# facebookresearch/vilbert-multi-task

Measured on AMD Instinct MI355X. Metric: samples/sec (36 regions, 36 tokens) ViLBERT-base 6L/6C fwd+bwd, higher is better.
Workload: dtype f32; 1 GPU; bert_base_6layer_6conect.json train_concap step: BertForMultiModalPreTraining fwd+bwd (dropout on) + grad all-reduce + AdamW, 36 regions + 1 global row, batch 256 per GPU, T=36 R=37; per_gpu_batch=256, global_batch=256, parallelism=dp1, visible_gpus=1, launch=eager, gemm_mode=f32, deterministic_wgrad=True, deterministic_fallbacks=0

## Files before the change

vilbert-multi-task_amd/csrc/common.h:

```cpp
#pragma once
#include <hip/hip_runtime.h>
#include <stdint.h>

#include "bf16_round.h"
#include "gemm_plan.h"
#include "row_checks.h"

typedef float f32x4 __attribute__((ext_vector_type(4)));
typedef float f32x16 __attribute__((ext_vector_type(16)));

#define VB_LAUNCH_CHECK()                         \
    do {                                          \
        hipError_t e__ = hipGetLastError();       \
        if (e__ != hipSuccess) return (int)e__;   \
    } while (0)

const uint64_t* vb_seed_epoch();

namespace vbemb {
int text_embed_bwd_det(hipStream_t st, int batch, int n_tok, int hidden, int vocab, int n_types, int n_tasks,
                       const int64_t* ids, const int64_t* seg, const int64_t* task_ids, const float* dx, float* dword,
                       float* dpos, float* dtype, float* dtask);
}

namespace vbrows {
int gather(hipStream_t st, long M, int cols, const float* src, const int32_t* map, long src_rows, float* out);
int drop_add(hipStream_t st, long M, int cols, const float* lin, const float* res, bool res_mapped, const int32_t* map,
             long src_rows, float* out, float p, uint64_t seed);
int invert(hipStream_t st, long src_rows, long M, const int32_t* map, int32_t* inv);
int scatter(hipStream_t st, long src_rows, int cols, const float* compact, long M, const int32_t* inv, float* full);
int move_rows(hipStream_t st, long rows, int chunks, const void* src, long lds, long src_rows, const int32_t* map, void* out,
              long ldo, long max_blocks);
int colsum_finish(hipStream_t st, long parts, int n, const float* part, long ldp, float* out);
}

__device__ __forceinline__ float wave_sum(float v) {
#pragma unroll
    for (int off = 32; off > 0; off >>= 1) v += __shfl_xor(v, off, 64);
    return v;
}

__device__ __forceinline__ void gelu_parts(float x, float& phi, float& e) {
    const float z = fabsf(x) * 0.70710678118654752440f;
    const float t = __builtin_amdgcn_rcpf(fmaf(0.3275911f, z, 1.0f));
    e = __expf(-z * z);
    float poly = fmaf(1.061405429f, t, -1.453152027f);
    poly = fmaf(poly, t, 1.421413741f);
    poly = fmaf(poly, t, -0.284496736f);
    poly = fmaf(poly, t, 0.254829592f);
    const float half_erfc = 0.5f * poly * t * e;
    phi = x >= 0.f ? 1.0f - half_erfc : half_erfc;
}

__device__ __forceinline__ float gelu_erf(float x) {
    float phi, e;
    gelu_parts(x, phi, e);
    return x * phi;
}

__device__ __forceinline__ float gelu_grad(float x) {
    float phi, e;
    gelu_parts(x, phi, e);
    return fmaf(x * 0.39894228040143267794f, e, phi);
}

__device__ __forceinline__ void gelu_and_grad(float x, float& y, float& d) {
    float phi, e;
    gelu_parts(x, phi, e);
    y = x * phi;
    d = fmaf(x * 0.39894228040143267794f, e, phi);
}

__device__ __forceinline__ float swish_act(float x) {
    return x / (1.0f + expf(-x));
}

__device__ __forceinline__ float swish_grad(float x) {
    const float s = 1.0f / (1.0f + expf(-x));
    return s + x * s * (1.0f - s);
}
```

vilbert-multi-task_amd/csrc/layernorm.hip:

```cpp
#include "rowops.h"
#include "rng.h"

using namespace vbrow;

namespace {

template <int NV>
__global__ __launch_bounds__(256) void layernorm_kernel(long rows, int n_cols, const float* __restrict__ x,
                                                        const float* __restrict__ x2,
                                                        const float* __restrict__ gamma,
                                                        const float* __restrict__ beta, float eps,
                                                        float* __restrict__ y, float* mean, float* rstd,
                                                        unsigned char* __restrict__ q, long ldq,
                                                        float* __restrict__ qscale, unsigned* __restrict__ mxs,
                                                        long mxs_rows) {
    const int lane = threadIdx.x & 63;
    const long row = (long)blockIdx.x * ROWS_PER_BLOCK + (threadIdx.x >> 6);
    if (row >= rows) return;
    const float* xr = x + row * n_cols;
    f32x4 v[NV];
#pragma unroll
    for (int i = 0; i < NV; ++i) {
        const int col = VB_LANE_COL(i, lane);
        v[i] = f32x4{0.f, 0.f, 0.f, 0.f};
        if (col < n_cols) {
            v[i] = *reinterpret_cast<const f32x4*>(xr + col);
            if (x2 != nullptr) v[i] += *reinterpret_cast<const f32x4*>(x2 + row * n_cols + col);
        }
    }
    ln_finish<NV>(v, n_cols, lane, gamma, beta, eps, y + row * n_cols, mean ? mean + row : nullptr,
                  rstd ? rstd + row : nullptr, nullptr, q ? q + row * ldq : nullptr, (q && qscale) ? qscale + row : nullptr,
                  mxs ? mxs + row : nullptr, mxs_rows);
}

struct EmitStats {
    static constexpr bool MX = false;
    float* __restrict__ mean;
    float* __restrict__ rstd;
};
struct EmitMX {
    static constexpr bool MX = true;
    unsigned char* __restrict__ q;
    long ldq;
    unsigned* __restrict__ mxs;
    long mxs_rows;
};

__device__ __forceinline__ f32x4 ln16_value(const uint2 w, const f32x4 g, const f32x4 b, float mean, float rstd) {
    return g * ((RowBF16::unpack(w) - mean) * rstd) + b;
}

template <int NV, int R, typename Emit>
__global__ __launch_bounds__(256) void layernorm16_kernel(long rows, int n_cols, const unsigned short* __restrict__ x,
                                                          const float* __restrict__ gamma, const float* __restrict__ beta,
                                                          float eps, unsigned short* __restrict__ y, const Emit out) {
    using IO = RowBF16;
    const int lane = threadIdx.x & 63;
    const long row0 = ((long)blockIdx.x * ROWS_PER_BLOCK + (threadIdx.x >> 6)) * R;
    if (row0 >= rows) return;
    long rrow[R];
    bool have[R];
#pragma unroll
    for (int r = 0; r < R; ++r) {
        have[r] = row0 + r < rows;
        rrow[r] = have[r] ? row0 + r : row0;
    }
    uint2 w[R][NV];
#pragma unroll
    for (int r = 0; r < R; ++r)
#pragma unroll
        for (int i = 0; i < NV; ++i) {
            const int col = VB_LANE_COL(i, lane);
            w[r][i] = uint2{0u, 0u};
            if (col < n_cols) w[r][i] = *reinterpret_cast<const uint2*>(x + rrow[r] * n_cols + col);
        }
    auto opaque = [&]() {
#pragma unroll
        for (int r = 0; r < R; ++r)
#pragma unroll
            for (int i = 0; i < NV; ++i) asm volatile("" : "+v"(w[r][i].x), "+v"(w[r][i].y));
    };
    float mu[R], q[R];
#pragma unroll
    for (int r = 0; r < R; ++r) {
        mu[r] = 0.f;
#pragma unroll
        for (int i = 0; i < NV; ++i) {
            const f32x4 v = IO::unpack(w[r][i]);
            mu[r] += (v[0] + v[1]) + (v[2] + v[3]);
        }
    }
    wave_sum_rows(mu);
    if (R > 1) opaque();
#pragma unroll
    for (int r = 0; r < R; ++r) {
        mu[r] /= (float)n_cols;
        q[r] = 0.f;
#pragma unroll
        for (int i = 0; i < NV; ++i) {
            const int col = VB_LANE_COL(i, lane);
            if (col < n_cols) {
                const f32x4 d = IO::unpack(w[r][i]) - mu[r];
                q[r] += (d[0] * d[0] + d[1] * d[1]) + (d[2] * d[2] + d[3] * d[3]);
            }
        }
    }
    wave_sum_rows(q);
    if (R > 1) opaque();
    if constexpr (!Emit::MX) {
#pragma unroll
        for (int r = 0; r < R; ++r) {
            q[r] = 1.0f / sqrtf(q[r] / (float)n_cols + eps);
            if (lane == 0 && have[r]) {
                if (out.mean != nullptr) out.mean[rrow[r]] = mu[r];
                if (out.rstd != nullptr) out.rstd[rrow[r]] = q[r];
            }
        }
#pragma unroll
        for (int i = 0; i < NV; ++i) {
            const int col = VB_LANE_COL(i, lane);
            if (col < n_cols) {
                const f32x4 g = *reinterpret_cast<const f32x4*>(gamma + col), b = *reinterpret_cast<const f32x4*>(beta + col);
#pragma unroll
                for (int r = 0; r < R; ++r)
                    if (have[r]) IO::store(y + rrow[r] * n_cols + col, ln16_value(w[r][i], g, b, mu[r], q[r]));
            }
        }
    } else {
        const int nkt = n_cols >> 7;
#pragma unroll
        for (int i = 0; i < NV; ++i) {
            const int col = VB_LANE_COL(i, lane);
            const bool ok = col < n_cols;
            f32x4 g = f32x4{0.f, 0.f, 0.f, 0.f}, b = f32x4{0.f, 0.f, 0.f, 0.f};
            if (ok) {
                g = *reinterpret_cast<const f32x4*>(gamma + col);
                b = *reinterpret_cast<const f32x4*>(beta + col);
            }
            const int kt = 2 * i + (lane >> 5);
#pragma unroll
            for (int r = 0; r < R; ++r) {
                const float rstd = 1.0f / sqrtf(q[r] / (float)n_cols + eps);
                const bool live = ok && have[r];
                f32x4 v = IO::unpack(w[r][i]);
                if (ok) v = ln16_value(w[r][i], g, b, mu[r], rstd);
                if (live) IO::store(y + rrow[r] * n_cols + col, v);
                mx_quant_chunk(v, live, lane, have[r] ? kt : nkt, nkt,
                               reinterpret_cast<unsigned*>(out.q + rrow[r] * out.ldq + (ok ? col : 0)),
                               out.mxs + (long)(kt < nkt ? kt : 0) * out.mxs_rows + rrow[r]);
            }
        }
    }
}

constexpr int LNB_ROWS_PER_WAVE = 4;
constexpr int LNB_ROWS_PER_BLOCK = 4 * LNB_ROWS_PER_WAVE;

inline long lnb_blocks(long rows) { return (rows + LNB_ROWS_PER_BLOCK - 1) / LNB_ROWS_PER_BLOCK; }

template <int NV, typename IO>
__global__ __launch_bounds__(256) void layernorm_bwd_kernel(long rows, int n_cols, const typename IO::elem* __restrict__ dy,
                                                            const typename IO::elem* __restrict__ x,
                                                            const float* __restrict__ mean, const float* __restrict__ rstd,
                                                            const float* __restrict__ gamma,
                                                            typename IO::elem* __restrict__ dx, float* __restrict__ ws,
                                                            typename IO::elem* __restrict__ dxd, float drop_p,
                                                            float drop_scale, uint64_t seed_in,
                                                            const uint64_t* __restrict__ epoch) {
    const uint64_t seed = dxd != nullptr ? vb_seed_with_epoch(seed_in, epoch) : 0;
    const int lane = threadIdx.x & 63, wave = threadIdx.x >> 6;
    const long part = (long)blockIdx.x * 4 + wave;
    const long row_begin = part * LNB_ROWS_PER_WAVE;
    f32x4 gam[NV], dg[NV], db[NV];
#pragma unroll
    for (int i = 0; i < NV; ++i) {
        const int col = VB_LANE_COL(i, lane);
        gam[i] = col < n_cols ? *reinterpret_cast<const f32x4*>(gamma + col) : f32x4{0.f, 0.f, 0.f, 0.f};
        dg[i] = f32x4{0.f, 0.f, 0.f, 0.f};
        db[i] = f32x4{0.f, 0.f, 0.f, 0.f};
    }
    [[maybe_unused]] typename IO::packed ndy[NV], nx[NV];
    [[maybe_unused]] float nmu = 0.f, nrs = 0.f;
    [[maybe_unused]] auto fetch = [&](long row) {
#pragma unroll
        for (int i = 0; i < NV; ++i) {
            const int col = VB_LANE_COL(i, lane);
            ndy[i] = IO::zero();
            nx[i] = IO::zero();
            if (col < n_cols) {
                ndy[i] = *reinterpret_cast<const typename IO::packed*>(dy + row * n_cols + col);
                nx[i] = *reinterpret_cast<const typename IO::packed*>(x + row * n_cols + col);
            }
        }
        nmu = mean[row];
        nrs = rstd[row];
    };
    if constexpr (IO::PREFETCH)
        if (row_begin < rows) fetch(row_begin);
    for (int rr = 0; rr < LNB_ROWS_PER_WAVE; ++rr) {
        const long row = row_begin + rr;
        if (row >= rows) break;
        const float mu = IO::PREFETCH ? nmu : mean[row], rs = IO::PREFETCH ? nrs : rstd[row];
        f32x4 xh[NV], g[NV];
        [[maybe_unused]] f32x4 dcur[NV];
        if constexpr (IO::PREFETCH) {
#pragma unroll
            for (int i = 0; i < NV; ++i) {
                dcur[i] = IO::unpack(ndy[i]);
                xh[i] = IO::unpack(nx[i]);
            }
            if (rr + 1 < LNB_ROWS_PER_WAVE && row + 1 < rows) fetch(row + 1);
        }
        float s1 = 0.f, s2 = 0.f;
#pragma unroll
        for (int i = 0; i < NV; ++i) {
            const int col = VB_LANE_COL(i, lane);
            if constexpr (!IO::PREFETCH) xh[i] = f32x4{0.f, 0.f, 0.f, 0.f};
            g[i] = f32x4{0.f, 0.f, 0.f, 0.f};
            if (col < n_cols) {
                const f32x4 d = IO::PREFETCH ? dcur[i] : *reinterpret_cast<const f32x4*>(dy + row * n_cols + col);
                xh[i] = ((IO::PREFETCH ? xh[i] : *reinterpret_cast<const f32x4*>(x + row * n_cols + col)) - mu) * rs;
                g[i] = d * gam[i];
                dg[i] += d * xh[i];
                db[i] += d;
                s1 += (g[i][0] + g[i][1]) + (g[i][2] + g[i][3]);
                s2 += (g[i][0] * xh[i][0] + g[i][1] * xh[i][1]) + (g[i][2] * xh[i][2] + g[i][3] * xh[i][3]);
            }
        }
        const float m1 = wave_sum(s1) / (float)n_cols, m2 = wave_sum(s2) / (float)n_cols;
#pragma unroll
        for (int i = 0; i < NV; ++i) {
            const int col = VB_LANE_COL(i, lane);
            if (col < n_cols) {
                const f32x4 d = (g[i] - m1 - xh[i] * m2) * rs;
                IO::store(dx + row * n_cols + col, d);
                if (dxd != nullptr) {
                    f32x4 dd;
                    const uint64_t idx = (uint64_t)(row * n_cols + col);
#pragma unroll
                    for (int e = 0; e < 4; ++e) dd[e] = vb_keep(seed, idx + e, drop_p) ? d[e] * drop_scale : 0.f;
                    IO::store(dxd + row * n_cols + col, dd);
                }
            }
        }
    }
    constexpr bool BLOCK_REDUCE = NV <= 4;
    __shared__ f32x4 red[BLOCK_REDUCE ? 3 * 2 * NV * 64 : 1];
    if (BLOCK_REDUCE) {
        if (wave > 0) {
#pragma unroll
            for (int i = 0; i < NV; ++i) {
                red[((wave - 1) * 2 * NV + i) * 64 + lane] = dg[i];
                red[((wave - 1) * 2 * NV + NV + i) * 64 + lane] = db[i];
            }
        }
        __syncthreads();
        if (wave > 0) return;
#pragma unroll
        for (int w2 = 0; w2 < 3; ++w2)
#pragma unroll
            for (int i = 0; i < NV; ++i) {
                dg[i] += red[(w2 * 2 * NV + i) * 64 + lane];
                db[i] += red[(w2 * 2 * NV + NV + i) * 64 + lane];
            }
    }
    float* w = ws + (BLOCK_REDUCE ? (long)blockIdx.x : part) * 2 * n_cols;
#pragma unroll
    for (int i = 0; i < NV; ++i) {
        const int col = VB_LANE_COL(i, lane);
        if (col < n_cols) {
            *reinterpret_cast<f32x4*>(w + col) = dg[i];
            *reinterpret_cast<f32x4*>(w + n_cols + col) = db[i];
        }
    }
}

__global__ __launch_bounds__(256) void layernorm_bwd_wide_kernel(long rows, int n_cols, const float* __restrict__ dy,
                                                                 const float* __restrict__ x,
                                                                 const float* __restrict__ mean,
                                                                 const float* __restrict__ rstd,
                                                                 const float* __restrict__ gamma,
                                                                 float* __restrict__ dx, float* __restrict__ ws) {
    const int lane = threadIdx.x & 63;
    const long row = (long)blockIdx.x * 4 + (threadIdx.x >> 6);
    if (row >= rows) return;
    const float mu = mean[row], rs = rstd[row];
    const float* __restrict__ dyr = dy + row * n_cols;
    const float* __restrict__ xr = x + row * n_cols;
    float s1 = 0.f, s2 = 0.f;
    for (int col = lane * 4; col < n_cols; col += 256) {
        const f32x4 d = *reinterpret_cast<const f32x4*>(dyr + col);
        const f32x4 xh = (*reinterpret_cast<const f32x4*>(xr + col) - mu) * rs;
        const f32x4 g = d * *reinterpret_cast<const f32x4*>(gamma + col);
        s1 += (g[0] + g[1]) + (g[2] + g[3]);
        s2 += (g[0] * xh[0] + g[1] * xh[1]) + (g[2] * xh[2] + g[3] * xh[3]);
    }
    const float m1 = wave_sum(s1) / (float)n_cols, m2 = wave_sum(s2) / (float)n_cols;
    float* __restrict__ w = ws + row * 2 * n_cols;
    for (int col = lane * 4; col < n_cols; col += 256) {
        const f32x4 d = *reinterpret_cast<const f32x4*>(dyr + col);
        const f32x4 xh = (*reinterpret_cast<const f32x4*>(xr + col) - mu) * rs;
        const f32x4 g = d * *reinterpret_cast<const f32x4*>(gamma + col);
        *reinterpret_cast<f32x4*>(dx + row * n_cols + col) = (g - m1 - xh * m2) * rs;
        *reinterpret_cast<f32x4*>(w + col) = d * xh;
        *reinterpret_cast<f32x4*>(w + n_cols + col) = d;
    }
}

template <int INFLIGHT>
__global__ __launch_bounds__(1024) void colreduce_kernel(long parts, int width, const float* __restrict__ ws,
                                                         float* __restrict__ out0, float* __restrict__ out1, int n_cols) {
    static_assert(INFLIGHT == 1 || INFLIGHT == 4, "instantiated forms");
    __shared__ float red[16][INFLIGHT == 1 ? 64 : 65];
    const int c = threadIdx.x & 63, pg = threadIdx.x >> 6;
    const int col = blockIdx.x * 64 + c;
    float s0 = 0.f, s1 = 0.f, s2 = 0.f, s3 = 0.f;
    if (col < width) {
        long p = pg;
        if constexpr (INFLIGHT == 4)
            for (; p + 48 < parts; p += 64) {
                s0 += ws[p * width + col];
                s1 += ws[(p + 16) * width + col];
                s2 += ws[(p + 32) * width + col];
                s3 += ws[(p + 48) * width + col];
            }
        for (; p < parts; p += 16) s0 += ws[p * width + col];
    }
    red[pg][c] = INFLIGHT == 4 ? (s0 + s1) + (s2 + s3) : s0;
    __syncthreads();
    if (pg == 0 && col < width) {
        float t = 0.f;
#pragma unroll
        for (int i = 0; i < 16; ++i) t += red[i][c];
        if (col < n_cols) out0[col] = t;
        else out1[col - n_cols] = t;
    }
}

template <int INFLIGHT>
int launch_colreduce(hipStream_t st, long parts, int n_cols, const float* ws, float* dgamma, float* dbeta) {
    const int width = 2 * n_cols;
    hipLaunchKernelGGL(colreduce_kernel<INFLIGHT>, dim3((unsigned)((width + 63) / 64)), dim3(1024), 0, st, parts, width, ws,
                       dgamma, dbeta, n_cols);
    VB_LAUNCH_CHECK();
    return 0;
}

inline bool codes_ok(const void* q, int64_t ldq, int n_cols) { return ldq >= n_cols && ldq % 4 == 0 && all_aligned(4, {q}); }

int launch_layernorm(void* stream, int64_t rows, int32_t n_cols, const float* x, const float* x2, const float* gamma,
                     const float* beta, float eps, float* y, float* mean, float* rstd, uint8_t* q, int64_t ldq,
                     float* qscale, uint32_t* mxs, int64_t mxs_rows) {
    if (!all_aligned(16, {x, x2, y, gamma, beta}) || (q != nullptr && !codes_ok(q, ldq, n_cols)) || !all_aligned(4, {mxs}))
        return VB_E_ALIGN;
    const dim3 grid((unsigned)((rows + ROWS_PER_BLOCK - 1) / ROWS_PER_BLOCK)), block(256);
    dispatch_nv<32>(nv_for(n_cols), [&](auto nv) {
        hipLaunchKernelGGL((layernorm_kernel<decltype(nv)::value>), grid, block, 0, static_cast<hipStream_t>(stream), (long)rows,
                           n_cols, x, x2, gamma, beta, eps, y, mean, rstd, q, (long)ldq, qscale, mxs, (long)mxs_rows);
    });
    VB_LAUNCH_CHECK();
    return 0;
}

template <int R, int MAX, typename Emit>
void launch_layernorm16(void* stream, int64_t rows, int32_t n_cols, const uint16_t* x, const float* gamma, const float* beta,
                        float eps, uint16_t* y, const Emit out) {
    const dim3 grid((unsigned)((rows + R * ROWS_PER_BLOCK - 1) / (R * ROWS_PER_BLOCK))), block(256);
    dispatch_nv<MAX>(nv_for(n_cols), [&](auto nv) {
        hipLaunchKernelGGL((layernorm16_kernel<decltype(nv)::value, R, Emit>), grid, block, 0, static_cast<hipStream_t>(stream),
                           (long)rows, n_cols, x, gamma, beta, eps, y, out);
    });
}

template <typename IO, int MAX, int INFLIGHT>
int layernorm_bwd_impl(void* stream, int64_t rows, int32_t n_cols, const typename IO::elem* dy, const typename IO::elem* x,
                       const float* mean, const float* rstd, const float* gamma, typename IO::elem* dx, float* dgamma,
                       float* dbeta, float* workspace, typename IO::elem* dxd, float drop_p, uint64_t seed) {
    if (!all_aligned(IO::ALIGN, {dy, x, dx, dxd}) || !all_aligned(16, {gamma, workspace})) return VB_E_ALIGN;
    hipStream_t st = static_cast<hipStream_t>(stream);
    const long blocks = lnb_blocks(rows);
    const float dscale = dxd != nullptr ? 1.0f / (1.0f - drop_p) : 1.0f;
    const uint64_t* epoch = vb_seed_epoch();
    dispatch_nv<MAX>(nv_for(n_cols), [&](auto nv) {
        hipLaunchKernelGGL((layernorm_bwd_kernel<decltype(nv)::value, IO>), dim3((unsigned)blocks), dim3(256), 0, st, (long)rows,
                           n_cols, dy, x, mean, rstd, gamma, dx, workspace, dxd, drop_p, dscale, seed, epoch);
    });
    VB_LAUNCH_CHECK();
    return launch_colreduce<INFLIGHT>(st, nv_for(n_cols) <= 4 ? blocks : blocks * 4, n_cols, workspace, dgamma, dbeta);
}

int layernorm_bwd_f32(void* stream, int64_t rows, int32_t n_cols, const float* dy, const float* x, const float* mean,
                      const float* rstd, const float* gamma, float* dx, float* dgamma, float* dbeta, float* workspace,
                      float* dxd, float drop_p, uint64_t seed) {
    if (any_null({dy, x, mean, rstd, gamma, dx, dgamma, dbeta, workspace}) || rows <= 0) return VB_E_BADARG;
    if (int e = check_cols(n_cols)) return e;
    if (nv_for(n_cols) <= 16)
        return layernorm_bwd_impl<RowF32, 16, 1>(stream, rows, n_cols, dy, x, mean, rstd, gamma, dx, dgamma, dbeta, workspace,
                                                 dxd, drop_p, seed);
    if (!all_aligned(16, {dy, x, dx, gamma, workspace})) return VB_E_ALIGN;
    if (dxd != nullptr) return VB_E_RANGE;
    hipStream_t st = static_cast<hipStream_t>(stream);
    hipLaunchKernelGGL(layernorm_bwd_wide_kernel, dim3((unsigned)((rows + 3) / 4)), dim3(256), 0, st, (long)rows, n_cols, dy, x,
                       mean, rstd, gamma, dx, workspace);
    VB_LAUNCH_CHECK();
    return launch_colreduce<1>(st, rows, n_cols, workspace, dgamma, dbeta);
}

}

extern "C" int vb_layernorm_fwd(void* stream, int64_t rows, int32_t n_cols, const float* x, const float* x2,
                                const float* gamma, const float* beta, float eps, float* y, float* mean,
                                float* rstd) {
    if (any_null({x, gamma, beta, y}) || rows <= 0) return VB_E_BADARG;
    if (int e = check_cols(n_cols)) return e;
    return launch_layernorm(stream, rows, n_cols, x, x2, gamma, beta, eps, y, mean, rstd, nullptr, 0, nullptr, nullptr, 0);
}

extern "C" int vb_layernorm_fwd_fp8(void* stream, int64_t rows, int32_t n_cols, const float* x, const float* x2,
                                    const float* gamma, const float* beta, float eps, float* y, uint8_t* q,
                                    int64_t ldq, float* qscale) {
    if (any_null({x, gamma, beta, y, q, qscale}) || rows <= 0) return VB_E_BADARG;
    if (int e = check_cols(n_cols)) return e;
    return launch_layernorm(stream, rows, n_cols, x, x2, gamma, beta, eps, y, nullptr, nullptr, q, ldq, qscale, nullptr, 0);
}

extern "C" int vb_layernorm_fwd_mx(void* stream, int64_t rows, int32_t n_cols, const float* x, const float* x2,
                                   const float* gamma, const float* beta, float eps, float* y, uint8_t* q, int64_t ldq,
                                   uint32_t* scales, int64_t scale_rows) {
    if (any_null({x, gamma, beta, y, q, scales}) || rows <= 0) return VB_E_BADARG;
    if (int e = check_cols(n_cols)) return e;
    if (n_cols % 128 != 0 || scale_rows < rows) return VB_E_RANGE;
    return launch_layernorm(stream, rows, n_cols, x, x2, gamma, beta, eps, y, nullptr, nullptr, q, ldq, nullptr, scales,
                            scale_rows);
}

extern "C" int vb_layernorm_fwd_mx16(void* stream, int64_t rows, int32_t n_cols, const uint16_t* x, const float* gamma,
                                     const float* beta, float eps, uint16_t* y, uint8_t* q, int64_t ldq, uint32_t* scales,
                                     int64_t scale_rows) {
    if (any_null({x, gamma, beta, y, q, scales}) || rows <= 0) return VB_E_BADARG;
    if (int e = check_cols(n_cols)) return e;
    if (n_cols % 128 != 0 || scale_rows < rows) return VB_E_RANGE;
    if (!all_aligned(RowBF16::ALIGN, {x, y}) || !all_aligned(16, {gamma, beta}) || !codes_ok(q, ldq, n_cols) ||
        !all_aligned(4, {scales}))
        return VB_E_ALIGN;
    const EmitMX out{q, (long)ldq, scales, (long)scale_rows};
    if ((rows + 2 * ROWS_PER_BLOCK - 1) / (2 * ROWS_PER_BLOCK) <= 2048 || n_cols > 1024)
        launch_layernorm16<2, 32>(stream, rows, n_cols, x, gamma, beta, eps, y, out);
    else
        launch_layernorm16<4, 4>(stream, rows, n_cols, x, gamma, beta, eps, y, out);
    VB_LAUNCH_CHECK();
    return 0;
}

extern "C" int vb_layernorm_fwd_bf16(void* stream, int64_t rows, int32_t n_cols, const uint16_t* x, const float* gamma,
                                     const float* beta, float eps, uint16_t* y, float* mean, float* rstd) {
    if (any_null({x, gamma, beta, y}) || rows <= 0) return VB_E_BADARG;
    if (n_cols <= 0 || n_cols % 4 != 0 || n_cols > 1024) return VB_E_RANGE;
    if (!all_aligned(RowBF16::ALIGN, {x, y}) || !all_aligned(16, {gamma, beta})) return VB_E_ALIGN;
    const EmitStats out{mean, rstd};
    if (rows < 4096) launch_layernorm16<1, 4>(stream, rows, n_cols, x, gamma, beta, eps, y, out);
    else if ((rows + 7) / 8 <= 2048) launch_layernorm16<2, 4>(stream, rows, n_cols, x, gamma, beta, eps, y, out);
    else launch_layernorm16<4, 4>(stream, rows, n_cols, x, gamma, beta, eps, y, out);
    VB_LAUNCH_CHECK();
    return 0;
}

extern "C" int64_t vb_layernorm_bwd_workspace(int64_t rows, int32_t n_cols) {
    if (rows <= 0 || n_cols <= 0) return 0;
    if (nv_for(n_cols) > 16) return rows * 2 * n_cols;
    const int64_t parts = (rows + LNB_ROWS_PER_WAVE - 1) / LNB_ROWS_PER_WAVE;
    const int64_t parts_padded = (parts + 3) / 4 * 4;
    return parts_padded * 2 * n_cols;
}

extern "C" int vb_layernorm_bwd(void* stream, int64_t rows, int32_t n_cols, const float* dy, const float* x,
                                const float* mean, const float* rstd, const float* gamma, float* dx,
                                float* dgamma, float* dbeta, float* workspace) {
    return layernorm_bwd_f32(stream, rows, n_cols, dy, x, mean, rstd, gamma, dx, dgamma, dbeta, workspace, nullptr, 0.f, 0);
}

extern "C" int vb_layernorm_bwd_drop(void* stream, int64_t rows, int32_t n_cols, const float* dy, const float* x,
                                     const float* mean, const float* rstd, const float* gamma, float* dx,
                                     float* dgamma, float* dbeta, float* workspace, float* dx_dropped, float dropout_p,
                                     uint64_t seed) {
    if (dx_dropped == nullptr || !(dropout_p > 0.f && dropout_p < 1.f)) return VB_E_BADARG;
    if (!vb_aligned16(dx_dropped)) return VB_E_ALIGN;
    return layernorm_bwd_f32(stream, rows, n_cols, dy, x, mean, rstd, gamma, dx, dgamma, dbeta, workspace, dx_dropped,
                             dropout_p, seed);
}

extern "C" int64_t vb_layernorm_bwd_bf16_workspace(int64_t rows, int32_t n_cols) {
    return lnb_blocks(rows) * 2 * (int64_t)n_cols;
}

extern "C" int vb_layernorm_bwd_bf16(void* stream, int64_t rows, int32_t n_cols, const uint16_t* dy, const uint16_t* x,
                                     const float* mean, const float* rstd, const float* gamma, uint16_t* dx, float* dgamma,
                                     float* dbeta, float* workspace, uint16_t* dx_dropped, float dropout_p, uint64_t seed) {
    if (any_null({dy, x, mean, rstd, gamma, dx, dgamma, dbeta, workspace}) || rows <= 0) return VB_E_BADARG;
    if (n_cols <= 0 || n_cols % 4 != 0 || n_cols > 1024) return VB_E_RANGE;
    if (dx_dropped != nullptr && !(dropout_p > 0.f && dropout_p < 1.f)) return VB_E_BADARG;
    return layernorm_bwd_impl<RowBF16, 4, 4>(stream, rows, n_cols, dy, x, mean, rstd, gamma, dx, dgamma, dbeta, workspace,
                                             dx_dropped, dropout_p, seed);
}
```

vilbert-multi-task_amd/csrc/layers.hip:

```cpp
#include "common.h"
#include "row_map.h"
#include <mutex>
#include <unordered_map>

namespace {

constexpr bool kF32 = false, kB16 = true;

#define VB_TRY(expr)               \
    do {                           \
        const int _e = (expr);     \
        if (_e != 0) return _e;    \
    } while (0)

template <bool B16>
struct Elem { static constexpr size_t size = B16 ? 2 : 4; };

template <bool B16>
inline const void* col(const void* p, long c) { return static_cast<const char*>(p) + c * (long)Elem<B16>::size; }
template <bool B16>
inline void* col(void* p, long c) { return static_cast<char*>(p) + c * (long)Elem<B16>::size; }

bool has_bias(const vb_layer_linear& L) { return L.bias[0] != nullptr; }
bool wants_wgrad(const vb_layer_linear& L) { return L.dw[0] != nullptr; }
// ... 118 lines not shown
        a.Q = static_cast<const uint16_t*>(c.q); a.ldq = c.ldq;
        a.K = static_cast<const uint16_t*>(c.k); a.ldk = c.ldk;
        a.V = static_cast<const uint16_t*>(c.v); a.ldv = c.ldk;
        a.mask_add = c.mask; a.O = static_cast<uint16_t*>(c.out); a.ldo = c.ldo; a.lse = c.lse;
        a.scale = scale; a.dropout_p = c.p; a.seed = c.seed;
        return vb_attention_fwd_bf16(st, &a);
    }
    vb_attention_args a{};
    a.batch = c.batch; a.heads = c.heads; a.head_dim = c.d; a.n_q = c.n_q; a.n_k = c.n_k;
    a.q_batch = c.batch; a.kv_batch = c.batch;
    a.Q = static_cast<const float*>(c.q); a.ldq = c.ldq;
    a.K = static_cast<const float*>(c.k); a.ldk = c.ldk;
    a.V = static_cast<const float*>(c.v); a.ldv = c.ldk;
    a.mask_add = c.mask; a.O = static_cast<float*>(c.out); a.ldo = c.ldo; a.lse = c.lse;
    a.scale = scale; a.dropout_p = c.p; a.seed = c.seed;
    return vb_attention_fwd(st, &a);
}

template <bool B16>
int attn_bwd(void* st, const AttnCall& c, const void* d_out, void* dq, void* dk, void* dv, long lddq, long lddk, float* dvec) {
    const float scale = (float)(1.0 / sqrt((double)c.d));
    if (B16) {
        vb_attention_bf16_args a{};
        a.batch = c.batch; a.heads = c.heads; a.head_dim = c.d; a.n_q = c.n_q; a.n_k = c.n_k;
        a.q_batch = c.batch; a.kv_batch = c.batch;
        a.Q = static_cast<const uint16_t*>(c.q); a.ldq = c.ldq;
        a.K = static_cast<const uint16_t*>(c.k); a.ldk = c.ldk;
        a.V = static_cast<const uint16_t*>(c.v); a.ldv = c.ldk;
        a.mask_add = c.mask; a.lse = c.lse; a.scale = scale; a.dropout_p = c.p; a.seed = c.seed;
        vb_attention_bf16_grads g{};
        g.dO = static_cast<const uint16_t*>(d_out); g.lddo = c.ldo;
        g.dQ = static_cast<uint16_t*>(dq); g.lddq = lddq;
        g.dK = static_cast<uint16_t*>(dk); g.lddk = lddk;
        g.dV = static_cast<uint16_t*>(dv); g.lddv = lddk;
        g.dvec = dvec;
        return vb_attention_bwd_bf16(st, &a, &g);
    }
    vb_attention_args a{};
    a.batch = c.batch; a.heads = c.heads; a.head_dim = c.d; a.n_q = c.n_q; a.n_k = c.n_k;
    a.q_batch = c.batch; a.kv_batch = c.batch;
    a.Q = static_cast<const float*>(c.q); a.ldq = c.ldq;
    a.K = static_cast<const float*>(c.k); a.ldk = c.ldk;
    a.V = static_cast<const float*>(c.v); a.ldv = c.ldk;
    a.mask_add = c.mask; a.lse = c.lse; a.scale = scale; a.dropout_p = c.p; a.seed = c.seed;
    vb_attention_grads g{};
    g.dO = static_cast<const float*>(d_out); g.lddo = c.ldo;
    g.dQ = static_cast<float*>(dq); g.lddq = lddq;
    g.dK = static_cast<float*>(dk); g.lddk = lddk;
    g.dV = static_cast<float*>(dv); g.lddv = lddk;
    g.dvec = dvec;
    return vb_attention_bwd(st, &a, &g);
}

std::mutex g_ev_mutex;
std::unordered_map<void*, hipEvent_t> g_fork_events;

int fork_to(void* main_st, void* side_st) {
    hipEvent_t ev;
    {
        std::lock_guard<std::mutex> lock(g_ev_mutex);
        auto it = g_fork_events.find(main_st);
        if (it == g_fork_events.end()) {
            const hipError_t e = hipEventCreateWithFlags(&ev, hipEventDisableTiming);
            if (e != hipSuccess) return (int)e;
            g_fork_events.emplace(main_st, ev);
        } else {
            ev = it->second;
        }
    }
    hipError_t e = hipEventRecord(ev, static_cast<hipStream_t>(main_st));
    if (e != hipSuccess) return (int)e;
    e = hipStreamWaitEvent(static_cast<hipStream_t>(side_st), ev, 0);
    return e == hipSuccess ? 0 : (int)e;
}

struct WgradJob { long M; const vb_layer_linear* L; const void* dY; const void* X; };
struct WgradQueue {
    WgradJob job[8];
    int n = 0;
    void push(long M, const vb_layer_linear& L, const void* dY, const void* X) {
        if (wants_wgrad(L) && n < 8) job[n++] = WgradJob{M, &L, dY, X};
    }
};

template <bool B16>
int wgrad_flush(void* st, void* side, const WgradQueue& q) {
    if (q.n == 0) return 0;
    void* target = st;
    if (side != nullptr && side != st) {
        VB_TRY(fork_to(st, side));
        target = side;
    }
    for (int i = 0; i < q.n; ++i) VB_TRY(wgrad<B16>(target, q.job[i].M, *q.job[i].L, q.job[i].dY, q.job[i].X));
    return 0;
}

AttnCall self_call(const vb_attn_block& b, bool b16) {
    const long Hb = (long)b.heads * b.head_dim, es = b16 ? 2 : 4;
    AttnCall c{};
    c.batch = b.batch; c.heads = b.heads; c.d = b.head_dim; c.n_q = b.n1; c.n_k = b.n1;
    c.q = b.qkv1_out;
    c.k = static_cast<const char*>(b.qkv1_out) + Hb * es;
    c.v = static_cast<const char*>(b.qkv1_out) + 2 * Hb * es;
    c.ldq = c.ldk = 3 * Hb;
    c.mask = b.mask1; c.out = b.ctx1; c.ldo = Hb; c.lse = b.lse1; c.p = b.p1; c.seed = b.seed1;
    return c;
}
AttnCall cross_call(const vb_attn_block& b, bool b16, int which) {
    const long Hb = (long)b.heads * b.head_dim, es = b16 ? 2 : 4;
    const void* qsrc = which == 1 ? b.qkv2_out : b.qkv1_out;
    const void* ksrc = which == 1 ? b.qkv1_out : b.qkv2_out;
    AttnCall c{};
    c.batch = b.batch; c.heads = b.heads; c.d = b.head_dim;
    c.n_q = which == 1 ? b.n2 : b.n1;
    c.n_k = which == 1 ? b.n1 : b.n2;
    c.q = qsrc;
    c.k = static_cast<const char*>(ksrc) + Hb * es;
    c.v = static_cast<const char*>(ksrc) + 2 * Hb * es;
    c.ldq = c.ldk = 3 * Hb;
    c.mask = which == 1 ? b.mask1 : b.mask2;
    c.out = which == 1 ? b.ctx1 : b.ctx2;
    c.ldo = Hb;
    c.lse = which == 1 ? b.lse1 : b.lse2;
    c.p = which == 1 ? b.p1 : b.p2;
    c.seed = which == 1 ? b.seed1 : b.seed2;
    return c;
}

template <bool B16>
int attn_block_fwd(void* st, const vb_attn_block& b) {
    const long M1 = (long)b.batch * b.n1;
    VB_TRY(linear<B16>(st, M1, b.qkv1, b.x1, b.qkv1_out, VB_ACT_NONE, nullptr, 0.f, 0, nullptr));
    if (b.n2 == 0) return attn_fwd<B16>(st, self_call(b, B16));
    const long M2 = (long)b.batch * b.n2;
    VB_TRY(linear<B16>(st, M2, b.qkv2, b.x2, b.qkv2_out, VB_ACT_NONE, nullptr, 0.f, 0, nullptr));
    VB_TRY(attn_fwd<B16>(st, cross_call(b, B16, 1)));
    return attn_fwd<B16>(st, cross_call(b, B16, 2));
}

int ffn_block_rows_fwd(void* st, const vb_ffn_block& f, bool training) {
    hipStream_t hs = static_cast<hipStream_t>(st);
    const long M = f.M, R = f.src_rows;
    float *sum1 = static_cast<float*>(f.sum1), *sum2 = static_cast<float*>(f.sum2);
    VB_TRY(vbrows::gather(hs, M, f.Hc, static_cast<const float*>(f.ctx), f.row_map, R, static_cast<float*>(f.ctx_rows)));
    VB_TRY(linear<kF32>(st, M, f.o, f.ctx_rows, sum1, VB_ACT_NONE, nullptr, 0.f, 0, nullptr));
    VB_TRY(vbrows::drop_add(hs, M, f.H, sum1, static_cast<const float*>(f.x), true, f.row_map, R, sum1, f.p_o, f.seed_o));
    VB_TRY(ln_fwd<kF32>(st, M, f.H, sum1, f.ln1, f.eps, f.a1, training ? f.mean1 : nullptr, training ? f.rstd1 : nullptr));
    VB_TRY(linear<kF32>(st, M, f.f1, f.a1, f.h, VB_ACT_GELU, nullptr, 0.f, 0, training ? f.dact : nullptr));
    VB_TRY(linear<kF32>(st, M, f.f2, f.h, sum2, VB_ACT_NONE, nullptr, 0.f, 0, nullptr));
    VB_TRY(vbrows::drop_add(hs, M, f.H, sum2, static_cast<const float*>(f.a1), false, f.row_map, R, sum2, f.p_f, f.seed_f));
    return ln_fwd<kF32>(st, M, f.H, sum2, f.ln2, f.eps, f.y, training ? f.mean2 : nullptr, training ? f.rstd2 : nullptr);
}

int ffn_block_rows_bwd(void* st, WgradQueue& wq, const vb_ffn_block& f) {
    hipStream_t hs = static_cast<hipStream_t>(st);
    const long M = f.M, R = f.src_rows;
    int32_t* inv = reinterpret_cast<int32_t*>(f.full_ws);
    auto compact = [](const void* p) { return static_cast<const float*>(p); };
    VB_TRY(ln_bwd<kF32>(st, M, f.H, f.dy, f.sum2, f.mean2, f.rstd2, f.ln2, f.d_sum2, f.ln_ws, nullptr, 0.f, 0));
    const void* dyd = f.d_sum2;
    if (f.p_f > 0.f) {
        VB_TRY(vbrows::drop_add(hs, M, f.H, compact(f.d_sum2), nullptr, false, f.row_map, R, static_cast<float*>(f.d_sum2_drop),
                                f.p_f, f.seed_f));
        dyd = f.d_sum2_drop;
    }
    VB_TRY(dgrad<kF32>(st, M, f.f2, dyd, f.d_pre, nullptr, f.dact));
    wq.push(M, f.f2, dyd, f.h);
    VB_TRY(dgrad<kF32>(st, M, f.f1, f.d_pre, f.d_a1, f.d_sum2, nullptr));
    wq.push(M, f.f1, f.d_pre, f.a1);
    VB_TRY(ln_bwd<kF32>(st, M, f.H, f.d_a1, f.sum1, f.mean1, f.rstd1, f.ln1, f.d_sum1, f.ln_ws, nullptr, 0.f, 0));
    const void* dod = f.d_sum1;
    if (f.p_o > 0.f) {
        VB_TRY(vbrows::drop_add(hs, M, f.H, compact(f.d_sum1), nullptr, false, f.row_map, R, static_cast<float*>(f.d_sum1_drop),
                                f.p_o, f.seed_o));
        dod = f.d_sum1_drop;
    }
    VB_TRY(dgrad<kF32>(st, M, f.o, dod, f.d_ctx, nullptr, nullptr));
    wq.push(M, f.o, dod, f.ctx_rows);
    VB_TRY(vbrows::invert(hs, R, M, f.row_map, inv));
    VB_TRY(vbrows::scatter(hs, R, f.H, compact(f.d_sum1), M, inv, static_cast<float*>(f.d_sum1_full)));
    return vbrows::scatter(hs, R, f.Hc, compact(f.d_ctx), M, inv, static_cast<float*>(f.d_ctx_full));
}

template <bool B16>
int ffn_block_fwd(void* st, const vb_ffn_block& f, bool training) {
    if (f.M == 0) return 0;
    if (f.row_map != nullptr) return ffn_block_rows_fwd(st, f, training);
    VB_TRY(linear<B16>(st, f.M, f.o, f.ctx, f.sum1, VB_ACT_NONE, f.x, f.p_o, f.seed_o, nullptr));
    VB_TRY(ln_fwd<B16>(st, f.M, f.H, f.sum1, f.ln1, f.eps, f.a1, training ? f.mean1 : nullptr, training ? f.rstd1 : nullptr));
    VB_TRY(linear<B16>(st, f.M, f.f1, f.a1, f.h, VB_ACT_GELU, nullptr, 0.f, 0, training ? f.dact : nullptr));
    VB_TRY(linear<B16>(st, f.M, f.f2, f.h, f.sum2, VB_ACT_NONE, f.a1, f.p_f, f.seed_f, nullptr));
    return ln_fwd<B16>(st, f.M, f.H, f.sum2, f.ln2, f.eps, f.y, training ? f.mean2 : nullptr, training ? f.rstd2 : nullptr);
}

template <bool B16>
int ffn_block_bwd(void* st, WgradQueue& wq, const vb_ffn_block& f) {
    if (f.M == 0) return 0;
    if (f.row_map != nullptr) return ffn_block_rows_bwd(st, wq, f);
    VB_TRY(ln_bwd<B16>(st, f.M, f.H, f.dy, f.sum2, f.mean2, f.rstd2, f.ln2, f.d_sum2, f.ln_ws, f.d_sum2_drop, f.p_f, f.seed_f));
    const void* dyd = f.p_f > 0.f ? f.d_sum2_drop : f.d_sum2;
    VB_TRY(dgrad<B16>(st, f.M, f.f2, dyd, f.d_pre, nullptr, f.dact));
    wq.push(f.M, f.f2, dyd, f.h);
    VB_TRY(dgrad<B16>(st, f.M, f.f1, f.d_pre, f.d_a1, f.d_sum2, nullptr));
    wq.push(f.M, f.f1, f.d_pre, f.a1);
    VB_TRY(ln_bwd<B16>(st, f.M, f.H, f.d_a1, f.sum1, f.mean1, f.rstd1, f.ln1, f.d_sum1, f.ln_ws, f.d_sum1_drop, f.p_o, f.seed_o));
    const void* dod = f.p_o > 0.f ? f.d_sum1_drop : f.d_sum1;
    VB_TRY(dgrad<B16>(st, f.M, f.o, dod, f.d_ctx, nullptr, nullptr));
    wq.push(f.M, f.o, dod, f.ctx);
    return 0;
}

template <bool B16>
int attn_block_bwd(void* st, WgradQueue& wq, const vb_attn_block& b) {
    const long Hb = (long)b.heads * b.head_dim, M1 = (long)b.batch * b.n1;
    if (b.n2 == 0) {
        VB_TRY(attn_bwd<B16>(st, self_call(b, B16), b.d_ctx1, b.dqkv1, col<B16>(b.dqkv1, Hb), col<B16>(b.dqkv1, 2 * Hb), 3 * Hb,
                             3 * Hb, b.dvec));
    } else {
        VB_TRY(attn_bwd<B16>(st, cross_call(b, B16, 1), b.d_ctx1, b.dqkv2, col<B16>(b.dqkv1, Hb), col<B16>(b.dqkv1, 2 * Hb), 3 * Hb,
                             3 * Hb, b.dvec));
        VB_TRY(attn_bwd<B16>(st, cross_call(b, B16, 2), b.d_ctx2, b.dqkv1, col<B16>(b.dqkv2, Hb), col<B16>(b.dqkv2, 2 * Hb), 3 * Hb,
                             3 * Hb, b.dvec));
    }
    if (b.dx1 != nullptr) VB_TRY(dgrad<B16>(st, M1, b.qkv1, b.dqkv1, b.dx1, b.dres1, nullptr));
    wq.push(M1, b.qkv1, b.dqkv1, b.x1);
    if (b.n2 != 0) {
        const long M2 = (long)b.batch * b.n2;
        if (b.dx2 != nullptr) VB_TRY(dgrad<B16>(st, M2, b.qkv2, b.dqkv2, b.dx2, b.dres2, nullptr));
        wq.push(M2, b.qkv2, b.dqkv2, b.x2);
    }
    return 0;
}

bool bad_linear(const vb_layer_linear& L, bool b16) {
    if (L.nseg < 1 || L.nseg > VB_MAX_SEGMENTS || L.seg_n <= 0 || L.K <= 0) return true;
    if (b16) return L.w16 == nullptr;
    for (int s = 0; s < L.nseg; ++s)
        if (L.w[s] == nullptr) return true;
    return false;
}

int check(const vb_layer_args* a, bool backward) {
    if (a == nullptr) return VB_E_BADARG;
    if (a->dtype != VB_DT_F32 && a->dtype != VB_DT_BF16) return VB_E_BADARG;
    const bool b16 = a->dtype == VB_DT_BF16;
    const vb_attn_block& b = a->attn;
    const bool has_attn = b.batch != 0;
    if (!has_attn && a->s1.M == 0 && a->s2.M == 0) return VB_E_BADARG;
    if (has_attn) {
        if (b.batch < 0 || b.heads <= 0 || b.head_dim <= 0 || b.n1 <= 0 || b.n2 < 0) return VB_E_BADARG;
        if (b.x1 == nullptr || b.qkv1_out == nullptr || b.ctx1 == nullptr || bad_linear(b.qkv1, b16)) return VB_E_BADARG;
        if ((long)b.qkv1.nseg * b.qkv1.seg_n != 3L * b.heads * b.head_dim) return VB_E_SEGMENT;
        if (b.n2 > 0) {
            if (b.x2 == nullptr || b.qkv2_out == nullptr || b.ctx2 == nullptr || bad_linear(b.qkv2, b16)) return VB_E_BADARG;
            if ((long)b.qkv2.nseg * b.qkv2.seg_n != 3L * b.heads * b.head_dim) return VB_E_SEGMENT;
        }
    }
    for (const vb_ffn_block* f : {&a->s1, &a->s2}) {
        if (f->M == 0) continue;
        if (f->M < 0 || f->H <= 0 || f->I <= 0 || f->Hc <= 0) return VB_E_BADARG;
        if (bad_linear(f->o, b16) || bad_linear(f->f1, b16) || bad_linear(f->f2, b16)) return VB_E_BADARG;
        if (f->o.K != f->Hc || f->o.nseg * f->o.seg_n != f->H || f->f1.K != f->H || f->f1.nseg * f->f1.seg_n != f->I ||
            f->f2.K != f->I || f->f2.nseg * f->f2.seg_n != f->H)
            return VB_E_SEGMENT;
        if (f->ctx == nullptr || f->x == nullptr || f->sum1 == nullptr || f->a1 == nullptr || f->h == nullptr || f->sum2 == nullptr ||
            f->y == nullptr || f->ln1.gamma == nullptr || f->ln2.gamma == nullptr)
            return VB_E_BADARG;
        if (backward) {
            if (f->dy == nullptr || f->d_sum2 == nullptr || f->d_pre == nullptr || f->d_a1 == nullptr || f->d_sum1 == nullptr ||
                f->d_ctx == nullptr || f->ln_ws == nullptr || f->dact == nullptr || f->mean1 == nullptr || f->mean2 == nullptr ||
                f->ln1.dgamma == nullptr || f->ln2.dgamma == nullptr)
                return VB_E_BADARG;
            if ((f->p_f > 0.f && f->d_sum2_drop == nullptr) || (f->p_o > 0.f && f->d_sum1_drop == nullptr)) return VB_E_BADARG;
        }
        if (int e = vbrows::check_row_map(*f, b16, backward)) return e;
    }
    if (backward && has_attn &&
        (b.dqkv1 == nullptr || b.dvec == nullptr || b.d_ctx1 == nullptr || b.lse1 == nullptr ||
         (b.n2 > 0 && (b.dqkv2 == nullptr || b.d_ctx2 == nullptr || b.lse2 == nullptr))))
        return VB_E_BADARG;
    return 0;
}

template <bool B16>
int layer_fwd(void* st, const vb_layer_args* a) {
    if (a->attn.batch != 0) VB_TRY(attn_block_fwd<B16>(st, a->attn));
    VB_TRY(ffn_block_fwd<B16>(st, a->s1, a->training != 0));
    return ffn_block_fwd<B16>(st, a->s2, a->training != 0);
}

template <bool B16>
int layer_bwd(void* st, const vb_layer_args* a) {
    static const bool each = [] { const char* e = getenv("VB_WGRAD_FORK"); return e != nullptr && e[0] == 'e'; }();
    WgradQueue wq;
    VB_TRY(ffn_block_bwd<B16>(st, wq, a->s1));
    if (each) { VB_TRY(wgrad_flush<B16>(st, a->wgrad_stream, wq)); wq.n = 0; }
    VB_TRY(ffn_block_bwd<B16>(st, wq, a->s2));
    if (each) { VB_TRY(wgrad_flush<B16>(st, a->wgrad_stream, wq)); wq.n = 0; }
    if (a->attn.batch != 0) VB_TRY(attn_block_bwd<B16>(st, wq, a->attn));
    return wgrad_flush<B16>(st, a->wgrad_stream, wq);
}

}

extern "C" int vb_layer_fwd(void* stream, const vb_layer_args* a) {
    VB_TRY(check(a, false));
    return a->dtype == VB_DT_BF16 ? layer_fwd<kB16>(stream, a) : layer_fwd<kF32>(stream, a);
}

extern "C" int vb_layer_bwd(void* stream, const vb_layer_args* a) {
    VB_TRY(check(a, true));
    return a->dtype == VB_DT_BF16 ? layer_bwd<kB16>(stream, a) : layer_bwd<kF32>(stream, a);
}
```

vilbert-multi-task_amd/csrc/rowmap.hip:

```cpp
#include "common.h"
#include "rng.h"
#include "row_kit.h"
#include "row_map.h"

namespace {

__device__ __forceinline__ long source_row(const int32_t* __restrict__ map, long r, long src_rows) {
    const long s = map[r];
    return s >= 0 && s < src_rows ? s : -1;
}

__global__ __launch_bounds__(256) void move_rows_kernel(long rows, int chunks, const v4i* __restrict__ src, long lds,
                                                        long src_rows, const int32_t* __restrict__ map,
                                                        v4i* __restrict__ out, long ldo) {
    const long n = rows * chunks;
    for (long i = (long)blockIdx.x * 256 + threadIdx.x; i < n; i += (long)gridDim.x * 256) {
        const long r = i / chunks, c = i - r * chunks;
        const long s = source_row(map, r, src_rows);
        out[r * ldo + c] = s >= 0 ? src[s * lds + c] : v4i{0, 0, 0, 0};
    }
}

__global__ __launch_bounds__(256) void row_drop_add_kernel(long M, int cols4, const f32x4* lin, const f32x4* __restrict__ res,
                                                           int res_mapped, const int32_t* __restrict__ map, long src_rows,
                                                           f32x4* out, float p, float scale, uint64_t seed_in,
                                                           const uint64_t* __restrict__ epoch) {
    const uint64_t seed = p > 0.f ? vb_seed_with_epoch(seed_in, epoch) : 0;
    const long n = M * cols4;
    for (long i = (long)blockIdx.x * blockDim.x + threadIdx.x; i < n; i += (long)gridDim.x * blockDim.x) {
        const long r = i / cols4, c = i - r * cols4;
        const long s = source_row(map, r, src_rows);
        f32x4 o = {0.f, 0.f, 0.f, 0.f};
        if (s >= 0) {
            f32x4 v = lin[i];
            if (p > 0.f) {
                const uint64_t idx = (uint64_t)((s * cols4 + c) * 4);
#pragma unroll
                for (int e = 0; e < 4; ++e) v[e] = vb_keep(seed, idx + e, p) ? v[e] * scale : 0.f;
            }
            o = v;
            if (res != nullptr) o += res[(res_mapped ? s : r) * cols4 + c];
        }
        out[i] = o;
    }
}

__global__ __launch_bounds__(256) void invert_map_kernel(long src_rows, int M, const int32_t* __restrict__ map,
                                                         int32_t* __restrict__ inv) {
    const int lane = threadIdx.x & 63;
    const long R = (long)blockIdx.x * 4 + (threadIdx.x >> 6);
    if (R >= src_rows) return;
    int found = -1;
    for (int base = 0; base < M && found < 0; base += 64) {
        const int r = base + lane;
        const unsigned long long hits = __ballot(r < M && (long)map[r] == R);
        if (hits != 0) found = base + __ffsll(hits) - 1;
    }
    if (lane == 0) inv[R] = found;
}

constexpr long ROW_MAX_BLOCKS = 2048;

}

namespace vbrows {

int move_rows(hipStream_t st, long rows, int chunks, const void* src, long lds, long src_rows, const int32_t* map, void* out,
              long ldo, long max_blocks) {
    hipLaunchKernelGGL(move_rows_kernel, dim3(vb_grid_for(rows * chunks, 256, max_blocks)), dim3(256), 0, st, rows, chunks,
                       static_cast<const v4i*>(src), lds, src_rows, map, static_cast<v4i*>(out), ldo);
    VB_LAUNCH_CHECK();
    return 0;
}

int gather(hipStream_t st, long M, int cols, const float* src, const int32_t* map, long src_rows, float* out) {
    return move_rows(st, M, cols / 4, src, cols / 4, src_rows, map, out, cols / 4, ROW_MAX_BLOCKS);
}

int drop_add(hipStream_t st, long M, int cols, const float* lin, const float* res, bool res_mapped, const int32_t* map,
             long src_rows, float* out, float p, uint64_t seed) {
    hipLaunchKernelGGL(row_drop_add_kernel, dim3(vb_grid_for(M * (cols / 4), 256, ROW_MAX_BLOCKS)), dim3(256), 0, st, M, cols / 4,
                       reinterpret_cast<const f32x4*>(lin), reinterpret_cast<const f32x4*>(res), res_mapped ? 1 : 0, map, src_rows,
                       reinterpret_cast<f32x4*>(out), p, 1.0f / (1.0f - p), seed, p > 0.f ? vb_seed_epoch() : nullptr);
    VB_LAUNCH_CHECK();
    return 0;
}

int invert(hipStream_t st, long src_rows, long M, const int32_t* map, int32_t* inv) {
    hipLaunchKernelGGL(invert_map_kernel, dim3((unsigned)((src_rows + 3) / 4)), dim3(256), 0, st, src_rows, (int)M, map, inv);
    VB_LAUNCH_CHECK();
    return 0;
}

int scatter(hipStream_t st, long src_rows, int cols, const float* compact, long M, const int32_t* inv, float* full) {
    return move_rows(st, src_rows, cols / 4, compact, cols / 4, M, inv, full, cols / 4, ROW_MAX_BLOCKS);
}

}
```

Before: 2591 samples/s.

## Fuse row-mapped dropout into LayerNorm backward, batch colreduce loads, rewrite map inversion

Adds a MAPPED variant of the LayerNorm backward kernel that applies dropout keyed by the source row index, replacing the separate drop_add pass in the FFN row-compacted backward. The column reduction for the non-4-inflight path now issues 8 independent loads per iteration for more memory-level parallelism. The inverse row map kernel moves from a per-row ballot scan over all M entries to a block-sliced shared-memory scatter. Together these remove one elementwise pass per LayerNorm and an O(R*M) scan, at the cost of extra template variants and a write race if the map has duplicates.

Result: no change. 2594 samples/s, median of 6 (+0.1%).

```diff
diff --git a/vilbert-multi-task_amd/csrc/common.h b/vilbert-multi-task_amd/csrc/common.h
--- a/vilbert-multi-task_amd/csrc/common.h
+++ b/vilbert-multi-task_amd/csrc/common.h
@@ -28,6 +28,9 @@
 int drop_add(hipStream_t st, long M, int cols, const float* lin, const float* res, bool res_mapped, const int32_t* map,
              long src_rows, float* out, float p, uint64_t seed);
 int invert(hipStream_t st, long src_rows, long M, const int32_t* map, int32_t* inv);
+int layernorm_bwd_drop_rows(hipStream_t st, long M, int n_cols, const float* dy, const float* x, const float* mean,
+                            const float* rstd, const float* gamma, float* dx, float* dgamma, float* dbeta, float* workspace,
+                            float* dx_dropped, float p, uint64_t seed, const int32_t* map, long src_rows);
 int scatter(hipStream_t st, long src_rows, int cols, const float* compact, long M, const int32_t* inv, float* full);
 int move_rows(hipStream_t st, long rows, int chunks, const void* src, long lds, long src_rows, const int32_t* map, void* out,
               long ldo, long max_blocks);
diff --git a/vilbert-multi-task_amd/csrc/layernorm.hip b/vilbert-multi-task_amd/csrc/layernorm.hip
--- a/vilbert-multi-task_amd/csrc/layernorm.hip
+++ b/vilbert-multi-task_amd/csrc/layernorm.hip
@@ -158,7 +158,7 @@
 
 inline long lnb_blocks(long rows) { return (rows + LNB_ROWS_PER_BLOCK - 1) / LNB_ROWS_PER_BLOCK; }
 
-template <int NV, typename IO>
+template <int NV, typename IO, bool MAPPED>
 __global__ __launch_bounds__(256) void layernorm_bwd_kernel(long rows, int n_cols, const typename IO::elem* __restrict__ dy,
                                                             const typename IO::elem* __restrict__ x,
                                                             const float* __restrict__ mean, const float* __restrict__ rstd,
@@ -166,7 +166,8 @@
                                                             typename IO::elem* __restrict__ dx, float* __restrict__ ws,
                                                             typename IO::elem* __restrict__ dxd, float drop_p,
                                                             float drop_scale, uint64_t seed_in,
-                                                            const uint64_t* __restrict__ epoch) {
+                                                            const uint64_t* __restrict__ epoch,
+                                                            const int32_t* __restrict__ map, long src_rows) {
     const uint64_t seed = dxd != nullptr ? vb_seed_with_epoch(seed_in, epoch) : 0;
     const int lane = threadIdx.x & 63, wave = threadIdx.x >> 6;
     const long part = (long)blockIdx.x * 4 + wave;
@@ -228,6 +229,11 @@
             }
         }
         const float m1 = wave_sum(s1) / (float)n_cols, m2 = wave_sum(s2) / (float)n_cols;
+        long mrow = row;
+        if constexpr (MAPPED) {
+            mrow = map[row];
+            if (mrow < 0 || mrow >= src_rows) mrow = -1;
+        }
 #pragma unroll
         for (int i = 0; i < NV; ++i) {
             const int col = VB_LANE_COL(i, lane);
@@ -236,9 +242,10 @@
                 IO::store(dx + row * n_cols + col, d);
                 if (dxd != nullptr) {
                     f32x4 dd;
-                    const uint64_t idx = (uint64_t)(row * n_cols + col);
+                    const uint64_t idx = (uint64_t)(mrow * n_cols + col);
 #pragma unroll
                     for (int e = 0; e < 4; ++e) dd[e] = vb_keep(seed, idx + e, drop_p) ? d[e] * drop_scale : 0.f;
+                    if (MAPPED && mrow < 0) dd = f32x4{0.f, 0.f, 0.f, 0.f};
                     IO::store(dxd + row * n_cols + col, dd);
                 }
             }
@@ -307,6 +314,8 @@
     }
 }
 
+constexpr int COLRED_BATCH = 8;
+
 template <int INFLIGHT>
 __global__ __launch_bounds__(1024) void colreduce_kernel(long parts, int width, const float* __restrict__ ws,
                                                          float* __restrict__ out0, float* __restrict__ out1, int n_cols) {
@@ -324,7 +333,24 @@
                 s2 += ws[(p + 32) * width + col];
                 s3 += ws[(p + 48) * width + col];
             }
-        for (; p < parts; p += 16) s0 += ws[p * width + col];
+        else
+            for (; p + 16 * (COLRED_BATCH - 1) < parts; p += 16 * COLRED_BATCH) {
+                float v[COLRED_BATCH];
+#pragma unroll
+                for (int b = 0; b < COLRED_BATCH; ++b) v[b] = ws[(p + 16 * b) * width + col];
+#pragma unroll
+                for (int b = 0; b < COLRED_BATCH; ++b) s0 += v[b];
+            }
+        if constexpr (INFLIGHT == 4) {
+            for (; p < parts; p += 16) s0 += ws[p * width + col];
+        } else if (p < parts) {
+            float v[COLRED_BATCH - 1];
+#pragma unroll
+            for (int b = 0; b < COLRED_BATCH - 1; ++b) v[b] = p + 16 * b < parts ? ws[(p + 16 * b) * width + col] : 0.f;
+#pragma unroll
+            for (int b = 0; b < COLRED_BATCH - 1; ++b)
+                if (p + 16 * b < parts) s0 += v[b];
+        }
     }
     red[pg][c] = INFLIGHT == 4 ? (s0 + s1) + (s2 + s3) : s0;
     __syncthreads();
@@ -372,18 +398,20 @@
     });
 }
 
-template <typename IO, int MAX, int INFLIGHT>
+template <typename IO, int MAX, int INFLIGHT, bool MAPPED = false>
 int layernorm_bwd_impl(void* stream, int64_t rows, int32_t n_cols, const typename IO::elem* dy, const typename IO::elem* x,
                        const float* mean, const float* rstd, const float* gamma, typename IO::elem* dx, float* dgamma,
-                       float* dbeta, float* workspace, typename IO::elem* dxd, float drop_p, uint64_t seed) {
+                       float* dbeta, float* workspace, typename IO::elem* dxd, float drop_p, uint64_t seed,
+                       const int32_t* map = nullptr, long src_rows = 0) {
     if (!all_aligned(IO::ALIGN, {dy, x, dx, dxd}) || !all_aligned(16, {gamma, workspace})) return VB_E_ALIGN;
     hipStream_t st = static_cast<hipStream_t>(stream);
     const long blocks = lnb_blocks(rows);
     const float dscale = dxd != nullptr ? 1.0f / (1.0f - drop_p) : 1.0f;
     const uint64_t* epoch = vb_seed_epoch();
     dispatch_nv<MAX>(nv_for(n_cols), [&](auto nv) {
-        hipLaunchKernelGGL((layernorm_bwd_kernel<decltype(nv)::value, IO>), dim3((unsigned)blocks), dim3(256), 0, st, (long)rows,
-                           n_cols, dy, x, mean, rstd, gamma, dx, workspace, dxd, drop_p, dscale, seed, epoch);
+        hipLaunchKernelGGL((layernorm_bwd_kernel<decltype(nv)::value, IO, MAPPED>), dim3((unsigned)blocks), dim3(256), 0, st,
+                           (long)rows, n_cols, dy, x, mean, rstd, gamma, dx, workspace, dxd, drop_p, dscale, seed, epoch, map,
+                           src_rows);
     });
     VB_LAUNCH_CHECK();
     return launch_colreduce<INFLIGHT>(st, nv_for(n_cols) <= 4 ? blocks : blocks * 4, n_cols, workspace, dgamma, dbeta);
@@ -406,6 +434,19 @@
     return launch_colreduce<1>(st, rows, n_cols, workspace, dgamma, dbeta);
 }
 
+}
+
+int vbrows::layernorm_bwd_drop_rows(hipStream_t st, long M, int n_cols, const float* dy, const float* x, const float* mean,
+                                    const float* rstd, const float* gamma, float* dx, float* dgamma, float* dbeta,
+                                    float* workspace, float* dx_dropped, float p, uint64_t seed, const int32_t* map,
+                                    long src_rows) {
+    if (any_null({dy, x, mean, rstd, gamma, dx, dgamma, dbeta, workspace, dx_dropped}) || map == nullptr || M <= 0 ||
+        src_rows <= 0 || !(p > 0.f && p < 1.f))
+        return VB_E_BADARG;
+    if (int e = check_cols(n_cols)) return e;
+    if (nv_for(n_cols) > 16) return VB_E_RANGE;
+    return layernorm_bwd_impl<RowF32, 16, 1, true>(st, M, n_cols, dy, x, mean, rstd, gamma, dx, dgamma, dbeta, workspace,
+                                                   dx_dropped, p, seed, map, src_rows);
 }
 
 extern "C" int vb_layernorm_fwd(void* stream, int64_t rows, int32_t n_cols, const float* x, const float* x2,
diff --git a/vilbert-multi-task_amd/csrc/layers.hip b/vilbert-multi-task_amd/csrc/layers.hip
--- a/vilbert-multi-task_amd/csrc/layers.hip
+++ b/vilbert-multi-task_amd/csrc/layers.hip
@@ -294,29 +294,28 @@
     return ln_fwd<kF32>(st, M, f.H, sum2, f.ln2, f.eps, f.y, training ? f.mean2 : nullptr, training ? f.rstd2 : nullptr);
 }
 
+int ln_rows_bwd(hipStream_t hs, const vb_ffn_block& f, const void* dy, const void* x, const float* mean, const float* rstd,
+                const vb_layer_norm& n, void* dx, void* dx_drop, float p, uint64_t seed) {
+    if (p > 0.f)
+        return vbrows::layernorm_bwd_drop_rows(hs, f.M, f.H, static_cast<const float*>(dy), static_cast<const float*>(x), mean,
+                                               rstd, n.gamma, static_cast<float*>(dx), n.dgamma, n.dbeta, f.ln_ws,
+                                               static_cast<float*>(dx_drop), p, seed, f.row_map, f.src_rows);
+    return ln_bwd<kF32>(hs, f.M, f.H, dy, x, mean, rstd, n, dx, f.ln_ws, nullptr, 0.f, 0);
+}
+
 int ffn_block_rows_bwd(void* st, WgradQueue& wq, const vb_ffn_block& f) {
     hipStream_t hs = static_cast<hipStream_t>(st);
     const long M = f.M, R = f.src_rows;
     int32_t* inv = reinterpret_cast<int32_t*>(f.full_ws);
     auto compact = [](const void* p) { return static_cast<const float*>(p); };
-    VB_TRY(ln_bwd<kF32>(st, M, f.H, f.dy, f.sum2, f.mean2, f.rstd2, f.ln2, f.d_sum2, f.ln_ws, nullptr, 0.f, 0));
-    const void* dyd = f.d_sum2;
-    if (f.p_f > 0.f) {
-        VB_TRY(vbrows::drop_add(hs, M, f.H, compact(f.d_sum2), nullptr, false, f.row_map, R, static_cast<float*>(f.d_sum2_drop),
-                                f.p_f, f.seed_f));
-        dyd = f.d_sum2_drop;
-    }
+    VB_TRY(ln_rows_bwd(hs, f, f.dy, f.sum2, f.mean2, f.rstd2, f.ln2, f.d_sum2, f.d_sum2_drop, f.p_f, f.seed_f));
+    const void* dyd = f.p_f > 0.f ? f.d_sum2_drop : f.d_sum2;
     VB_TRY(dgrad<kF32>(st, M, f.f2, dyd, f.d_pre, nullptr, f.dact));
     wq.push(M, f.f2, dyd, f.h);
     VB_TRY(dgrad<kF32>(st, M, f.f1, f.d_pre, f.d_a1, f.d_sum2, nullptr));
     wq.push(M, f.f1, f.d_pre, f.a1);
-    VB_TRY(ln_bwd<kF32>(st, M, f.H, f.d_a1, f.sum1, f.mean1, f.rstd1, f.ln1, f.d_sum1, f.ln_ws, nullptr, 0.f, 0));
-    const void* dod = f.d_sum1;
-    if (f.p_o > 0.f) {
-        VB_TRY(vbrows::drop_add(hs, M, f.H, compact(f.d_sum1), nullptr, false, f.row_map, R, static_cast<float*>(f.d_sum1_drop),
-                                f.p_o, f.seed_o));
-        dod = f.d_sum1_drop;
-    }
+    VB_TRY(ln_rows_bwd(hs, f, f.d_a1, f.sum1, f.mean1, f.rstd1, f.ln1, f.d_sum1, f.d_sum1_drop, f.p_o, f.seed_o));
+    const void* dod = f.p_o > 0.f ? f.d_sum1_drop : f.d_sum1;
     VB_TRY(dgrad<kF32>(st, M, f.o, dod, f.d_ctx, nullptr, nullptr));
     wq.push(M, f.o, dod, f.ctx_rows);
     VB_TRY(vbrows::invert(hs, R, M, f.row_map, inv));
diff --git a/vilbert-multi-task_amd/csrc/rowmap.hip b/vilbert-multi-task_amd/csrc/rowmap.hip
--- a/vilbert-multi-task_amd/csrc/rowmap.hip
+++ b/vilbert-multi-task_amd/csrc/rowmap.hip
@@ -45,18 +45,22 @@
     }
 }
 
-__global__ __launch_bounds__(256) void invert_map_kernel(long src_rows, int M, const int32_t* __restrict__ map,
-                                                         int32_t* __restrict__ inv) {
-    const int lane = threadIdx.x & 63;
-    const long R = (long)blockIdx.x * 4 + (threadIdx.x >> 6);
-    if (R >= src_rows) return;
-    int found = -1;
-    for (int base = 0; base < M && found < 0; base += 64) {
-        const int r = base + lane;
-        const unsigned long long hits = __ballot(r < M && (long)map[r] == R);
-        if (hits != 0) found = base + __ffsll(hits) - 1;
+constexpr int INV_RANGE = 512;
+
+__global__ __launch_bounds__(INV_RANGE) void invert_map_kernel(long src_rows, int M, const int32_t* __restrict__ map,
+                                                               int32_t* __restrict__ inv) {
+    __shared__ int32_t slice[INV_RANGE];
+    const long base = (long)blockIdx.x * INV_RANGE;
+    const long count = src_rows - base < INV_RANGE ? src_rows - base : INV_RANGE;
+    slice[threadIdx.x] = -1;
+    __syncthreads();
+#pragma unroll 8
+    for (int r = threadIdx.x; r < M; r += INV_RANGE) {
+        const long at = (long)map[r] - base;
+        if (at >= 0 && at < count) slice[at] = r;
     }
-    if (lane == 0) inv[R] = found;
+    __syncthreads();
+    if (threadIdx.x < count) inv[base + threadIdx.x] = slice[threadIdx.x];
 }
 
 constexpr long ROW_MAX_BLOCKS = 2048;
@@ -87,7 +91,8 @@
 }
 
 int invert(hipStream_t st, long src_rows, long M, const int32_t* map, int32_t* inv) {
-    hipLaunchKernelGGL(invert_map_kernel, dim3((unsigned)((src_rows + 3) / 4)), dim3(256), 0, st, src_rows, (int)M, map, inv);
+    hipLaunchKernelGGL(invert_map_kernel, dim3((unsigned)((src_rows + INV_RANGE - 1) / INV_RANGE)), dim3(INV_RANGE), 0, st,
+                       src_rows, (int)M, map, inv);
     VB_LAUNCH_CHECK();
     return 0;
 }
```
